# allegro/allRank

Measured on NVIDIA H100. Metric: slates/sec, higher is better.
Workload: dtype tf32

## Files before the change

### allrank_b200/csrc/gemm_tf32.cu

```cuda
#include <cstdio>
#include <cstring>
#include <cuda.h>
#include <cuda_runtime.h>

#include "common.h"
#include "defaults.h"
#include "gemm_tf32.h"
#include "sm90_ptx.cuh"

namespace arb {

constexpr int BLOCK_M = 128;
constexpr int BLOCK_K = 32;
constexpr int BLOCK_K_BF16 = 64;
constexpr int A_STAGE_BYTES = BLOCK_M * BLOCK_K * 4;
constexpr int GEMM_EPI_GROUPS = 1;
constexpr int GEMM_EPI_THREADS = 128 * GEMM_EPI_GROUPS;
constexpr int GEMM_THREADS = 64 + GEMM_EPI_THREADS;
constexpr int XPOSE_BYTES = 32 * 33 * 4;

struct GemmParams {
  int M, N, K;
  int nb2;
  int a_b2, a_b3, b_b2, b_b3, c_b2, c_b3;
// ... 9 lines not shown
  float* colsum_out;
  const int* rows_dev;
  uint32_t* bits;
};

template <bool MN, bool IN16>
__device__ __forceinline__ uint32_t op_word(const uint8_t* s, int rc, int k, int rnd) {
  if constexpr (IN16) {
    if constexpr (MN) {
      const uint8_t* slab = s + (rc >> 6) * 8192;
      const uint32_t lo = *reinterpret_cast<const uint16_t*>(slab + ptx::sw128(k, 2 * (rc & 63)));
      const uint32_t hi = *reinterpret_cast<const uint16_t*>(slab + ptx::sw128(k + 1, 2 * (rc & 63)));
      return lo | (hi << 16);
    } else {
      return *reinterpret_cast<const uint32_t*>(s + ptx::sw128(rc, 2 * k));
    }
  } else {
    const float x = MN ? ptx::ld_f32(s + (rc >> 5) * 4096, k, rc & 31) : ptx::ld_f32(s, rc, k);
    return rnd ? ptx::cvt_tf32(x) : __float_as_uint(x);
  }
}

template <int NT, bool A_MN, bool B_MN, bool IN16>
__device__ __forceinline__ void warp_mma_kblock(float (&acc)[2][NT][4], const uint8_t* a_s, const uint8_t* b_s, int row0,
                                                int slab0, int slab_step, int rnd) {
  const int lane = threadIdx.x & 31, g = lane >> 2, t = lane & 3;
#pragma unroll
  for (int ks = 0; ks < 4; ++ks) {
    const int k0 = IN16 ? 16 * ks + 2 * t : 8 * ks + t;
    const int kh = IN16 ? 8 : 4;
    uint32_t a[2][4];
#pragma unroll
    for (int mt = 0; mt < 2; ++mt) {
      const int r = row0 + 16 * mt + g;
      a[mt][0] = op_word<A_MN, IN16>(a_s, r, k0, rnd);
      a[mt][1] = op_word<A_MN, IN16>(a_s, r + 8, k0, rnd);
      a[mt][2] = op_word<A_MN, IN16>(a_s, r, k0 + kh, rnd);
      a[mt][3] = op_word<A_MN, IN16>(a_s, r + 8, k0 + kh, rnd);
    }
#pragma unroll
    for (int nt = 0; nt < NT; ++nt) {
      const int n = 32 * (slab0 + slab_step * (nt >> 2)) + 8 * (nt & 3) + g;
      const uint32_t b[2] = {op_word<B_MN, IN16>(b_s, n, k0, rnd), op_word<B_MN, IN16>(b_s, n, k0 + kh, rnd)};
#pragma unroll
      for (int mt = 0; mt < 2; ++mt) {
        if constexpr (IN16) ptx::mma_bf16(acc[mt][nt], a[mt], b);
        else ptx::mma_tf32(acc[mt][nt], a[mt], b);
      }
    }
  }
}

template <int A_MN, int B_MN, bool IN16>
constexpr bool use_wgmma() { return A_MN == 0 && B_MN == 0 && !IN16; }
template <int BLOCK_N>
constexpr int wg_cols() { return BLOCK_N == 128 ? 64 : 32; }

template <int NT, int WN>
__device__ __forceinline__ void wg_mma_kblock(float (&acc)[2][NT][4], const uint8_t* a_s, uint8_t* b_s, int col0,
                                              int rnd, int rnd_b, int bar) {
  const int lane = threadIdx.x & 31, w = (threadIdx.x >> 5) & 3, j = lane >> 3;
  if (rnd_b) {
    float4* b4 = reinterpret_cast<float4*>(b_s + col0 * 128);
#pragma unroll
    for (int i = threadIdx.x & 127; i < NT * 8 * 8; i += 128) {
      float4 v = b4[i];
      v.x = __uint_as_float(ptx::cvt_tf32(v.x)); v.y = __uint_as_float(ptx::cvt_tf32(v.y));
      v.z = __uint_as_float(ptx::cvt_tf32(v.z)); v.w = __uint_as_float(ptx::cvt_tf32(v.w));
      b4[i] = v;
    }
    ptx::fence_proxy_async_smem();
    ptx::named_bar_sync(bar, 128);
  }
  uint32_t a[4][2][4];
#pragma unroll
  for (int ks = 0; ks < 4; ++ks)
#pragma unroll
    for (int mt = 0; mt < 2; ++mt) {
      ptx::ldmatrix_x4(a[ks][mt], a_s + ptx::sw128(64 * mt + 16 * w + 8 * (j & 1) + (lane & 7), 32 * ks + 16 * (j >> 1)));
      if (rnd) {
#pragma unroll
        for (int e = 0; e < 4; ++e) a[ks][mt][e] = ptx::cvt_tf32(__uint_as_float(a[ks][mt][e]));
      }
    }
  const uint64_t desc = ptx::wgmma_desc_sw128(b_s + col0 * 128);
  ptx::wgmma_fence_acc(acc[0]);
  ptx::wgmma_fence_acc(acc[1]);
  ptx::wgmma_fence();
#pragma unroll
  for (int ks = 0; ks < 4; ++ks)
#pragma unroll
    for (int mt = 0; mt < 2; ++mt) {
      const uint64_t d = desc + 2 * ks;
      if constexpr (WN == 64) {
        ptx::wgmma_m64n64k8_tf32<0>(acc[mt], a[ks][mt], d);
        if constexpr (NT == 16) ptx::wgmma_m64n64k8_tf32<8>(acc[mt], a[ks][mt], d + 64 * 128 / 16);
      } else {
        ptx::wgmma_m64n32k8_tf32<0>(acc[mt], a[ks][mt], d);
        if constexpr (NT == 8) ptx::wgmma_m64n32k8_tf32<4>(acc[mt], a[ks][mt], d + 32 * 128 / 16);
      }
    }
  ptx::wgmma_commit();
  ptx::wgmma_wait0();
  ptx::wgmma_fence_acc(acc[0]);
  ptx::wgmma_fence_acc(acc[1]);
}

template <int NT>
__device__ __forceinline__ void acc_chunk_row(const float (&acc)[2][NT][4], int c, float* xp, uint32_t (&v)[32]) {
  const int lane = threadIdx.x & 31, g = lane >> 2, t = lane & 3;
  __syncwarp();
#pragma unroll
  for (int cc = 0; cc < NT / 4; ++cc) {
    if (cc != c) continue;
#pragma unroll
    for (int mt = 0; mt < 2; ++mt)
#pragma unroll
      for (int j = 0; j < 4; ++j) {
        float* r0 = xp + (16 * mt + g) * 33 + 8 * j + 2 * t;
        r0[0] = acc[mt][4 * cc + j][0];
        r0[1] = acc[mt][4 * cc + j][1];
        r0[8 * 33] = acc[mt][4 * cc + j][2];
        r0[8 * 33 + 1] = acc[mt][4 * cc + j][3];
      }
  }
  __syncwarp();
#pragma unroll
  for (int j = 0; j < 32; ++j) v[j] = __float_as_uint(xp[lane * 33 + j]);
}

template <int F>
__device__ __forceinline__ uint32_t epi_chunk_f32(const uint32_t (&v)[32], uint8_t* slab_row, int row, const float* bias_c,
                                                  float alpha, uint32_t word = 0u) {
  uint32_t out_bits = 0u;
#pragma unroll
  for (int piece = 0; piece < 8; ++piece) {
    float4* dst = reinterpret_cast<float4*>(slab_row + ((piece ^ (row & 7)) << 4));
    float4 o = make_float4(__uint_as_float(v[piece * 4 + 0]) * alpha, __uint_as_float(v[piece * 4 + 1]) * alpha,
                           __uint_as_float(v[piece * 4 + 2]) * alpha, __uint_as_float(v[piece * 4 + 3]) * alpha);
    if constexpr ((F & EPI_BIAS) != 0) {
      const float4 bv = *reinterpret_cast<const float4*>(bias_c + 4 * piece);
      o.x += bv.x; o.y += bv.y; o.z += bv.z; o.w += bv.w;
    }
    if constexpr ((F & EPI_RELU) != 0) {
      o.x = fmaxf(o.x, 0.0f); o.y = fmaxf(o.y, 0.0f); o.z = fmaxf(o.z, 0.0f); o.w = fmaxf(o.w, 0.0f);
    }
    if constexpr ((F & (EPI_ADD_AUX | EPI_MASK_AUX)) != 0) {
      const float4 a = *dst;
      if constexpr ((F & EPI_ADD_AUX) != 0) { o.x += a.x; o.y += a.y; o.z += a.z; o.w += a.w; }
      if constexpr ((F & EPI_MASK_AUX) != 0) {
        o.x = a.x > 0.f ? o.x : 0.f; o.y = a.y > 0.f ? o.y : 0.f; o.z = a.z > 0.f ? o.z : 0.f; o.w = a.w > 0.f ? o.w : 0.f;
      }
    }
    if constexpr ((F & EPI_MASK_BITS) != 0) {
      o.x = (word >> (4 * piece + 0)) & 1u ? o.x : 0.f; o.y = (word >> (4 * piece + 1)) & 1u ? o.y : 0.f;
      o.z = (word >> (4 * piece + 2)) & 1u ? o.z : 0.f; o.w = (word >> (4 * piece + 3)) & 1u ? o.w : 0.f;
    }
    if constexpr ((F & EPI_RELU_BITS) != 0) {
      out_bits |= (o.x > 0.f ? 1u : 0u) << (4 * piece + 0) | (o.y > 0.f ? 1u : 0u) << (4 * piece + 1) |
                  (o.z > 0.f ? 1u : 0u) << (4 * piece + 2) | (o.w > 0.f ? 1u : 0u) << (4 * piece + 3);
    }
    *dst = o;
  }
  return out_bits;
}
__device__ __forceinline__ bool epi_chunk_dispatch(int flags, const uint32_t (&v)[32], uint8_t* slab_row, int row,
                                                   const float* bias_c, float alpha, uint32_t* bits_at = nullptr,
                                                   uint32_t word_in = 0u) {
  switch (flags & (EPI_BIAS | EPI_RELU | EPI_ADD_AUX | EPI_MASK_AUX | EPI_DROPOUT | EPI_ATOMIC | EPI_RELU_BITS | EPI_MASK_BITS)) {
    case 0: epi_chunk_f32<0>(v, slab_row, row, bias_c, alpha); return true;
    case EPI_BIAS: epi_chunk_f32<EPI_BIAS>(v, slab_row, row, bias_c, alpha); return true;
    case EPI_BIAS | EPI_RELU: epi_chunk_f32<EPI_BIAS | EPI_RELU>(v, slab_row, row, bias_c, alpha); return true;
    case EPI_BIAS | EPI_ADD_AUX: epi_chunk_f32<EPI_BIAS | EPI_ADD_AUX>(v, slab_row, row, bias_c, alpha); return true;
    case EPI_MASK_AUX: epi_chunk_f32<EPI_MASK_AUX>(v, slab_row, row, bias_c, alpha); return true;
    case EPI_BIAS | EPI_RELU | EPI_RELU_BITS: {
      const uint32_t w = epi_chunk_f32<EPI_BIAS | EPI_RELU | EPI_RELU_BITS>(v, slab_row, row, bias_c, alpha);
      if (bits_at) *bits_at = w;
      return true;
    }
    case EPI_MASK_BITS:
      epi_chunk_f32<EPI_MASK_BITS>(v, slab_row, row, bias_c, alpha, word_in);
      return true;
    default: return false;
  }
}

template <int BLOCK_N, int NST = 2>
struct SmemLayout {
  static constexpr int B_STAGE_BYTES = BLOCK_N * BLOCK_K * 4;
  static constexpr int STAGE_BYTES = A_STAGE_BYTES + B_STAGE_BYTES;
  static constexpr int STAGING_BYTES = BLOCK_M * BLOCK_N * 4;
  static constexpr int stages() { return NST; }
  static constexpr int pipe_bytes() { return stages() * STAGE_BYTES; }
  static constexpr int body_bytes() { return pipe_bytes() > STAGING_BYTES ? pipe_bytes() : STAGING_BYTES; }
  static constexpr int XPOSE_OFF = 256 + BLOCK_N * 4;
  static constexpr int total() { return body_bytes() + XPOSE_OFF + (GEMM_EPI_THREADS / 32) * XPOSE_BYTES + 1024; }
};

template <int BLOCK_N, int A_MN, int B_MN, bool DROP, int NST, bool IN16 = false, bool OUT16 = false>
__global__ void __launch_bounds__(GEMM_THREADS) gemm_tf32_kernel(const __grid_constant__ CUtensorMap tmA,
                                                                 const __grid_constant__ CUtensorMap tmB,
                                                                 const __grid_constant__ CUtensorMap tmC,
                                                                 const __grid_constant__ CUtensorMap tmAux,
                                                                 const GemmParams p) {
  using L = SmemLayout<BLOCK_N, NST>;
  constexpr int STAGES = L::stages();
  constexpr int N_SLABS = BLOCK_N / 32;
  constexpr int NT = BLOCK_N / 8;
  constexpr int N_CONSUMERS = GEMM_EPI_THREADS / 32;
  constexpr bool WG = use_wgmma<A_MN, B_MN, IN16>();
  constexpr int OUT_COLS = OUT16 ? 64 : 32;
  constexpr int OUT_SLABS = (BLOCK_N + OUT_COLS - 1) / OUT_COLS;
  static_assert(!OUT16 || BLOCK_N >= 64, "bf16 outputs need at least one full 128-byte slab row");

  extern __shared__ uint8_t smem_dyn[];
  uint8_t* smem = reinterpret_cast<uint8_t*>((reinterpret_cast<uintptr_t>(smem_dyn) + 1023) & ~uintptr_t(1023));
  const bool has_aux = (p.flags & (EPI_ADD_AUX | EPI_MASK_AUX)) != 0;
  uint8_t* staging = smem;
  uint8_t* tail = smem + L::body_bytes();
  uint64_t* full_bar = reinterpret_cast<uint64_t*>(tail);
  uint64_t* empty_bar = full_bar + STAGES;
  uint64_t* ring_done_bar = empty_bar + STAGES;
  uint64_t* aux_bar = ring_done_bar + 1;
  float* bias_s = reinterpret_cast<float*>(tail + 256);

  const int warp = threadIdx.x >> 5, lane = threadIdx.x & 31;
  const int n0 = blockIdx.x * BLOCK_N, m0 = blockIdx.y * BLOCK_M;
  const bool split = (p.flags & EPI_ATOMIC) != 0;
  const int b2 = split ? 0 : int(blockIdx.z) % p.nb2, b3 = split ? 0 : int(blockIdx.z) / p.nb2;
  constexpr int KELEMS = IN16 ? BLOCK_K_BF16 : BLOCK_K;
  constexpr int MN_SLAB = IN16 ? 64 : 32;
  constexpr int MN_SLAB_BYTES = MN_SLAB * KELEMS * (IN16 ? 2 : 4);
  const bool dev_rows = p.rows_dev != nullptr;
  if (dev_rows && !split && m0 >= __ldg(p.rows_dev)) return;
  const int k_live = (dev_rows && split) ? min(p.K, __ldg(p.rows_dev)) : p.K;
  const int total_kb = (k_live + KELEMS - 1) / KELEMS;
  const int kb_per = (dev_rows && split) ? (total_kb + int(gridDim.z) - 1) / int(gridDim.z) : p.kb_per_split;
  const int kb_begin = split ? int(blockIdx.z) * kb_per : 0;
  const int kb_end = split ? min(total_kb, kb_begin + kb_per) : total_kb;
  const int nkb = max(0, kb_end - kb_begin);

  if (warp == 0 && lane == 0) {
    ptx::prefetch_tmap(&tmA);
    ptx::prefetch_tmap(&tmB);
    if (!split) ptx::prefetch_tmap(&tmC);
    if (has_aux) ptx::prefetch_tmap(&tmAux);
    for (int s = 0; s < STAGES; ++s) { ptx::mbar_init(&full_bar[s], 1); ptx::mbar_init(&empty_bar[s], N_CONSUMERS); }
    ptx::mbar_init(ring_done_bar, N_CONSUMERS);
    ptx::mbar_init(aux_bar, 1);
    ptx::fence_barrier_init();
  }
  arb_pdl_wait();
  __syncthreads();

  if (warp == N_CONSUMERS) {
    if (lane == 0) {
      for (int i = 0; i < nkb; ++i) {
        const int s = i % STAGES, round = i / STAGES;
        if (round > 0) ptx::mbar_wait(&empty_bar[s], (round - 1) & 1);
        uint8_t* a_s = smem + s * L::STAGE_BYTES;
        uint8_t* b_s = a_s + A_STAGE_BYTES;
        const int k0 = (kb_begin + i) * KELEMS;
        ptx::mbar_expect_tx(&full_bar[s], L::STAGE_BYTES);
        if (A_MN) {
          for (int c = 0; c < BLOCK_M / MN_SLAB; ++c)
            ptx::tma_load_4d(a_s + c * MN_SLAB_BYTES, &tmA, &full_bar[s], m0 + MN_SLAB * c, k0, b2 * p.a_b2, b3 * p.a_b3);
        } else {
          ptx::tma_load_4d(a_s, &tmA, &full_bar[s], k0, m0, b2 * p.a_b2, b3 * p.a_b3);
        }
        if (B_MN) {
          for (int c = 0; c < BLOCK_N / MN_SLAB; ++c)
            ptx::tma_load_4d(b_s + c * MN_SLAB_BYTES, &tmB, &full_bar[s], n0 + MN_SLAB * c, k0, b2 * p.b_b2, b3 * p.b_b3);
        } else {
          ptx::tma_load_4d(b_s, &tmB, &full_bar[s], k0, n0, b2 * p.b_b2, b3 * p.b_b3);
        }
      }
      if (has_aux) {
        if (nkb > 0) ptx::mbar_wait(ring_done_bar, 0);
        ptx::mbar_expect_tx(aux_bar, OUT16 ? L::STAGING_BYTES / 2 : L::STAGING_BYTES);
        for (int c = 0; c < OUT_SLABS; ++c)
          ptx::tma_load_4d(staging + c * (BLOCK_M * 128), &tmAux, aux_bar, n0 + OUT_COLS * c, m0, b2 * p.c_b2, b3 * p.c_b3);
      }
    }
  } else if (warp < N_CONSUMERS) {
    const int q = warp & 3;
    const int row = WG ? 64 * (lane >> 4) + 16 * q + (lane & 15) : 32 * q + lane;
    const int et = threadIdx.x;
    const int grp = warp >> 2;
    float* xp = reinterpret_cast<float*>(tail + L::XPOSE_OFF) + warp * (XPOSE_BYTES / 4);
    if (p.flags & EPI_BIAS) {
      for (int j = et; j < BLOCK_N; j += GEMM_EPI_THREADS) bias_s[j] = (n0 + j < p.N) ? p.bias[n0 + j] : 0.0f;
    }
    auto mask_word = [&](int c) -> uint32_t {
      return ((p.flags & EPI_MASK_BITS) && c < N_SLABS && m0 + row < p.M && n0 + 32 * c < p.N)
                 ? p.bits[(long long)(m0 + row) * (p.N >> 5) + ((n0 >> 5) + c)] : 0u;
    };
    uint32_t word_next = mask_word(grp);
    float acc[2][NT][4];
#pragma unroll
    for (int mt = 0; mt < 2; ++mt)
#pragma unroll
      for (int nt = 0; nt < NT; ++nt) acc[mt][nt][0] = acc[mt][nt][1] = acc[mt][nt][2] = acc[mt][nt][3] = 0.f;
    for (int i = 0; i < nkb; ++i) {
      const int s = i % STAGES, round = i / STAGES;
      ptx::mbar_wait(&full_bar[s], round & 1);
      uint8_t* a_s = smem + s * L::STAGE_BYTES;
      if constexpr (WG) wg_mma_kblock<NT, wg_cols<BLOCK_N>()>(acc, a_s, a_s + A_STAGE_BYTES, 0, p.rnd, p.rnd_b, 1);
      else warp_mma_kblock<NT, A_MN, B_MN, IN16>(acc, a_s, a_s + A_STAGE_BYTES, 32 * q, 0, 1, p.rnd);
      __syncwarp();
      if (lane == 0) ptx::mbar_arrive(&empty_bar[s]);
    }
    if (lane == 0) ptx::mbar_arrive(ring_done_bar);
    ptx::named_bar_sync(1, GEMM_EPI_THREADS);
    if (has_aux) ptx::mbar_wait(aux_bar, 0);
#pragma unroll 1
    for (int c = grp; c < N_SLABS; c += GEMM_EPI_GROUPS) {
      const uint32_t word_in = word_next;
      word_next = mask_word(c + GEMM_EPI_GROUPS);
      uint32_t v[32];
      acc_chunk_row<NT>(acc, c, xp, v);
      if constexpr (OUT16) {
        uint8_t* slab_row = staging + (c >> 1) * (BLOCK_M * 128) + row * 128;
#pragma unroll
        for (int piece = 0; piece < 4; ++piece) {
          uint4* dst = reinterpret_cast<uint4*>(slab_row + ((((c & 1) * 4 + piece) ^ (row & 7)) << 4));
          float o[8];
#pragma unroll
          for (int e = 0; e < 8; ++e) {
            const int j = piece * 8 + e;
            float x = __uint_as_float(v[j]) * p.alpha;
            if (p.flags & EPI_BIAS) x += bias_s[32 * c + j];
            if (p.flags & EPI_RELU) x = fmaxf(x, 0.0f);
            if constexpr (DROP) {
              const unsigned long long idx = (unsigned long long)(m0 + row) * (unsigned long long)p.N + (n0 + 32 * c + j);
              x = drop_keep(idx, p.drop.seed, p.drop.thresh) ? x * p.drop.scale : 0.0f;
            }
            o[e] = x;
          }
          if (has_aux) {
            const uint4 a = *dst;
            const uint32_t w[4] = {a.x, a.y, a.z, a.w};
#pragma unroll
            for (int e = 0; e < 8; ++e) {
              const uint32_t h = (w[e >> 1] >> ((e & 1) * 16)) & 0xffffu;
              const float av = __uint_as_float(h << 16);
              if (p.flags & EPI_ADD_AUX) o[e] += av;
              if (p.flags & EPI_MASK_AUX) o[e] = av > 0.f ? o[e] : 0.f;
            }
          }
          uint4 pk;
          pk.x = ptx::pack_bf16(o[0], o[1]); pk.y = ptx::pack_bf16(o[2], o[3]);
          pk.z = ptx::pack_bf16(o[4], o[5]); pk.w = ptx::pack_bf16(o[6], o[7]);
          *dst = pk;
        }
        continue;
      }
      uint8_t* slab_row = staging + c * (BLOCK_M * 128) + row * 128;
      if constexpr (!DROP) {
        uint32_t* bits_at = (p.bits && m0 + row < p.M && n0 + 32 * c < p.N)
                                ? p.bits + (long long)(m0 + row) * (p.N >> 5) + ((n0 >> 5) + c) : nullptr;
        if (epi_chunk_dispatch(p.flags, v, slab_row, row, bias_s + 32 * c, p.alpha, bits_at, word_in)) continue;
      }
#pragma unroll
// ... 51 lines not shown
          const uint8_t* slab = staging + (et >> 6) * (BLOCK_M * 128);
          const int cc = et & 63;
#pragma unroll 8
          for (int r = 0; r < BLOCK_M; ++r) {
            const uint16_t hv = *reinterpret_cast<const uint16_t*>(slab + r * 128 + ((((cc >> 3) ^ (r & 7)) << 4) | ((cc & 7) << 1)));
            t += __uint_as_float(uint32_t(hv) << 16);
          }
        } else {
          const uint8_t* slab = staging + (et >> 5) * (BLOCK_M * 128);
          const int cc = et & 31;
#pragma unroll 8
          for (int r = 0; r < BLOCK_M; ++r)
            t += *reinterpret_cast<const float*>(slab + r * 128 + ((((cc >> 2) ^ (r & 7)) << 4) | ((cc & 3) << 2)));
        }
        p.colsum_out[((long long)blockIdx.z * gridDim.y + blockIdx.y) * p.N + n0 + et] = t;
      }
      if (et == 0) ptx::tma_store_wait_read();
    }
  }
  __syncthreads();
}

template <int BLOCK_N>
struct PersistLayout {
  static constexpr int B_STAGE_BYTES = BLOCK_N * BLOCK_K * 4;
  static constexpr int STAGE_BYTES = A_STAGE_BYTES + B_STAGE_BYTES;
  static constexpr int STAGES = BLOCK_N <= 64 ? 6 : 3;
  static constexpr int STAGING_BYTES = BLOCK_M * BLOCK_N * 4;
  static constexpr int RING_BYTES = STAGES * STAGE_BYTES;
  static constexpr int XPOSE_OFF = RING_BYTES + STAGING_BYTES + 512 + BLOCK_N * 4;
  static constexpr int total();
};

constexpr int EPI_GROUPS = 2;
constexpr int EPI_THREADS = 128 * EPI_GROUPS;
constexpr int PERSIST_THREADS = 64 + EPI_THREADS;
template <int BLOCK_N>
constexpr int PersistLayout<BLOCK_N>::total() { return XPOSE_OFF + (EPI_THREADS / 32) * XPOSE_BYTES + 1024; }

template <int BLOCK_N, int A_MN, int B_MN>
__global__ void __launch_bounds__(PERSIST_THREADS, 1) gemm_tf32_persistent(const __grid_constant__ CUtensorMap tmA,
                                                                        const __grid_constant__ CUtensorMap tmB,
                                                                        const __grid_constant__ CUtensorMap tmC,
                                                                        const __grid_constant__ CUtensorMap tmAux,
                                                                        const GemmParams p, int n_tiles_n,
                                                                        int n_tiles_m, int n_z) {
  using L = PersistLayout<BLOCK_N>;
  constexpr int STAGES = L::STAGES;
  constexpr int N_SLABS = BLOCK_N / 32;
  constexpr int NGA = N_SLABS < EPI_GROUPS ? N_SLABS : EPI_GROUPS;
  constexpr int SLABS_PER_GROUP = N_SLABS / NGA;
  constexpr int NT = 4 * SLABS_PER_GROUP;
  constexpr bool WG = use_wgmma<A_MN, B_MN, false>();
  static_assert(!WG || 32 * SLABS_PER_GROUP == wg_cols<BLOCK_N>(), "a group's columns are one wgmma instruction wide");
  constexpr int PRODUCER_WARP = EPI_THREADS / 32;

  extern __shared__ uint8_t smem_dyn[];
  uint8_t* smem = reinterpret_cast<uint8_t*>((reinterpret_cast<uintptr_t>(smem_dyn) + 1023) & ~uintptr_t(1023));
  uint8_t* staging = smem + L::RING_BYTES;
  uint64_t* full_bar = reinterpret_cast<uint64_t*>(staging + L::STAGING_BYTES);
  uint64_t* empty_bar = full_bar + STAGES;
  uint64_t* aux_full = empty_bar + STAGES;
  uint64_t* stage_free = aux_full + 1;
  float* bias_s = reinterpret_cast<float*>(staging + L::STAGING_BYTES + 512);

  const int warp = threadIdx.x >> 5, lane = threadIdx.x & 31;
  const bool split = (p.flags & EPI_ATOMIC) != 0;
  const bool has_aux = (p.flags & (EPI_ADD_AUX | EPI_MASK_AUX)) != 0;
  const bool dev_rows = p.rows_dev != nullptr;
  if (dev_rows && !split) n_tiles_m = min(n_tiles_m, (__ldg(p.rows_dev) + BLOCK_M - 1) / BLOCK_M);
  const int total_kb = (((dev_rows && split) ? min(p.K, __ldg(p.rows_dev)) : p.K) + BLOCK_K - 1) / BLOCK_K;
  const int kb_per = (dev_rows && split) ? (total_kb + n_z - 1) / n_z : p.kb_per_split;
  const int n_tiles = n_tiles_n * n_tiles_m * n_z;

  if (warp == 0 && lane == 0) {
    ptx::prefetch_tmap(&tmA);
    ptx::prefetch_tmap(&tmB);
    if (!split) ptx::prefetch_tmap(&tmC);
    if (has_aux) ptx::prefetch_tmap(&tmAux);
    for (int s = 0; s < STAGES; ++s) { ptx::mbar_init(&full_bar[s], 1); ptx::mbar_init(&empty_bar[s], 4 * NGA); }
    ptx::mbar_init(aux_full, 1);
    ptx::mbar_init(stage_free, NGA);
    ptx::fence_barrier_init();
  }
  arb_pdl_wait();
  __syncthreads();

  auto decode = [&](int t, int& n0, int& m0, int& z) {
    const int nt = t % n_tiles_n;
    const int rest = t / n_tiles_n;
    n0 = nt * BLOCK_N;
    m0 = (rest % n_tiles_m) * BLOCK_M;
    z = rest / n_tiles_m;
  };
  auto k_range = [&](int z, int& kb0, int& nkb) {
    if (split) {
      kb0 = z * kb_per;
      nkb = min(total_kb, kb0 + kb_per) - kb0;
      if (nkb < 0) nkb = 0;
    } else {
      kb0 = 0;
      nkb = total_kb;
    }
  };

  if (warp == PRODUCER_WARP) {
// ... 238 lines not shown
static int launch_persistent_t(const GemmDesc& d, const CUtensorMap& tA, const CUtensorMap& tB, const CUtensorMap& tC,
                               const CUtensorMap& tX, const GemmParams& p, dim3 tiles, cudaStream_t st) {
  const long long n_tiles = (long long)tiles.x * tiles.y * tiles.z;
  const int grid = int(std::min<long long>(n_tiles, sm_count()));
  const double nb = double(d.nb2) * double(d.nb3);
  const double has_x = (d.flags & (EPI_ADD_AUX | EPI_MASK_AUX)) ? 1.0 : 0.0;
  char pname[56];
  gemm_prof_name(pname, d, "persist");
  const double dM = live_m(d), dK = live_k(d);
  ProfScope ps(ARB_PROF_GEMM, 2.0 * dM * double(d.N) * dK * nb, st,
               4.0 * nb * (dM * dK + double(d.N) * dK + (1.0 + has_x) * dM * d.N), pname);
  return launch(gemm_tf32_persistent<BLOCK_N, A_MN, B_MN>, dim3(grid), dim3(PERSIST_THREADS),
                PersistLayout<BLOCK_N>::total(), st, true, tA, tB, tC, tX, p, int(tiles.x), int(tiles.y),
                int(tiles.z));
}

template <int BLOCK_N, int A_MN, int B_MN>
static int launch_bf16_t(const GemmDesc& d, const CUtensorMap& tA, const CUtensorMap& tB, const CUtensorMap& tC,
                         const CUtensorMap& tX, const GemmParams& p, dim3 grid, cudaStream_t st) {
  constexpr bool WGRAD = (A_MN == 1 && B_MN == 1);
  const bool drop = (p.flags & EPI_DROPOUT) != 0;
  if (drop && (A_MN || B_MN)) { arb_set_error("gemm_bf16: dropout epilogue needs K-major operands"); return ARB_E_UNSUPPORTED; }
  void (*kern)(CUtensorMap, CUtensorMap, CUtensorMap, CUtensorMap, GemmParams) = nullptr;
  int smem = 0;
  if constexpr (WGRAD) {
    kern = gemm_tf32_kernel<BLOCK_N, 1, 1, false, 4, true, false>; smem = SmemLayout<BLOCK_N, 4>::total();
  } else if constexpr (BLOCK_N >= 64) {
    constexpr bool CAN_DROP = (A_MN == 0 && B_MN == 0);
    if (d.C.bf16) {
      if (drop) kern = gemm_tf32_kernel<BLOCK_N, A_MN, B_MN, CAN_DROP, 3, true, true>;
      else      kern = gemm_tf32_kernel<BLOCK_N, A_MN, B_MN, false, 3, true, true>;
    } else {
      if (drop) kern = gemm_tf32_kernel<BLOCK_N, A_MN, B_MN, CAN_DROP, 3, true, false>;
      else      kern = gemm_tf32_kernel<BLOCK_N, A_MN, B_MN, false, 3, true, false>;
    }
    smem = SmemLayout<BLOCK_N, 3>::total();
  }
  if (!kern) { arb_set_error("gemm_bf16: block_n must be 64 or 128"); return ARB_E_UNSUPPORTED; }
  const double nb = double(d.nb2) * double(d.nb3);
  const double has_x = (d.flags & (EPI_ADD_AUX | EPI_MASK_AUX)) ? 1.0 : 0.0;
  const double osz = d.C.bf16 ? 2.0 : 4.0;
  char pname[56];
  gemm_prof_name(pname, d, "tile");
  const double dM = live_m(d), dK = live_k(d);
  ProfScope ps(ARB_PROF_GEMM, 2.0 * dM * double(d.N) * dK * nb, st,
               nb * (2.0 * (dM * dK + double(d.N) * dK) + osz * (1.0 + has_x) * dM * d.N), pname);
  return launch(kern, grid, dim3(GEMM_THREADS), smem, st, true, tA, tB, tC, tX, p);
}

template <int BLOCK_N, int A_MN, int B_MN>
static int launch_t(const GemmDesc& d, const CUtensorMap& tA, const CUtensorMap& tB, const CUtensorMap& tC,
                    const CUtensorMap& tX, const GemmParams& p, dim3 grid, cudaStream_t st) {
  if (d.A.bf16) return launch_bf16_t<BLOCK_N, A_MN, B_MN>(d, tA, tB, tC, tX, p, grid, st);
  const bool has_aux_tile = (p.flags & (EPI_ADD_AUX | EPI_MASK_AUX)) != 0;
  const bool pick = !(A_MN == 1 && B_MN == 1) && !(p.flags & EPI_ATOMIC) && d.nb2 == 1 && d.nb3 == 1 &&
                    (d.K >= 256 || !has_aux_tile || g_persistent == 3);
  if (g_persistent == 1 || (g_persistent >= 2 && pick))
    return launch_persistent_t<BLOCK_N, A_MN, B_MN>(d, tA, tB, tC, tX, p, grid, st);
  constexpr bool CAN_DROP = (A_MN == 0 && B_MN == 0);
  constexpr bool WGRAD = (A_MN == 1 && B_MN == 1);
  const bool drop = (p.flags & EPI_DROPOUT) != 0;
  if (drop && !CAN_DROP) { arb_set_error("gemm_tf32: dropout epilogue needs K-major operands"); return ARB_E_UNSUPPORTED; }
  const bool deep = !WGRAD && d.K >= 256;
  void (*kern)(CUtensorMap, CUtensorMap, CUtensorMap, CUtensorMap, GemmParams);
  int smem;
  if (WGRAD) {
    kern = gemm_tf32_kernel<BLOCK_N, A_MN, B_MN, false, 4>; smem = SmemLayout<BLOCK_N, 4>::total();
  } else if (drop) {
    if (deep) { kern = gemm_tf32_kernel<BLOCK_N, A_MN, B_MN, CAN_DROP, 3>; smem = SmemLayout<BLOCK_N, 3>::total(); }
    else      { kern = gemm_tf32_kernel<BLOCK_N, A_MN, B_MN, CAN_DROP, 2>; smem = SmemLayout<BLOCK_N, 2>::total(); }
  } else {
    if (deep) { kern = gemm_tf32_kernel<BLOCK_N, A_MN, B_MN, false, 3>; smem = SmemLayout<BLOCK_N, 3>::total(); }
    else      { kern = gemm_tf32_kernel<BLOCK_N, A_MN, B_MN, false, 2>; smem = SmemLayout<BLOCK_N, 2>::total(); }
  }
  const double nb = double(d.nb2) * double(d.nb3);
  const double has_x = (d.flags & (EPI_ADD_AUX | EPI_MASK_AUX)) ? 1.0 : 0.0;
  char pname[56];
  gemm_prof_name(pname, d, "tile");
  const double dM = live_m(d), dK = live_k(d);
  ProfScope ps(ARB_PROF_GEMM, 2.0 * dM * double(d.N) * dK * nb, st,
               4.0 * nb * (dM * dK + double(d.N) * dK + (1.0 + has_x) * dM * d.N), pname);
  return launch(kern, grid, dim3(GEMM_THREADS), smem, st, true, tA, tB, tC, tX, p);
}

int launch_gemm_tf32(const GemmDesc& d, cudaStream_t st) {
  if (d.M <= 0 || d.N <= 0 || d.K < 0) { arb_set_error("gemm_tf32: bad shape"); return ARB_E_INVALID_ARG; }
  if (d.block_n != 32 && d.block_n != 64 && d.block_n != 128) { arb_set_error("gemm_tf32: block_n must be 32/64/128"); return ARB_E_INVALID_ARG; }
  const bool split = (d.flags & EPI_ATOMIC) != 0;
  if (split && (d.nb2 != 1 || d.nb3 != 1 || !d.atomic_out)) { arb_set_error("gemm_tf32: split-K needs an unbatched problem and atomic_out"); return ARB_E_INVALID_ARG; }
  if (!split && d.split_k != 1) { arb_set_error("gemm_tf32: split_k > 1 needs EPI_ATOMIC"); return ARB_E_INVALID_ARG; }
  const bool in16 = d.A.bf16 != 0, out16 = d.C.bf16 != 0;
  if ((d.B.bf16 != 0) != in16) { arb_set_error("gemm: A and B must have the same element type"); return ARB_E_INVALID_ARG; }
  if (out16 && (!in16 || split || d.block_n < 64)) { arb_set_error("gemm: a bf16 output needs bf16 operands, no split-K and block_n >= 64"); return ARB_E_INVALID_ARG; }
  if ((d.flags & (EPI_ADD_AUX | EPI_MASK_AUX)) && (d.Aux.bf16 != 0) != out16) { arb_set_error("gemm: the aux tile must have the output's element type"); return ARB_E_INVALID_ARG; }
  if (in16 && d.block_n < 64) { arb_set_error("gemm: bf16 operands need block_n >= 64 (a 128-byte row holds 64 elements)"); return ARB_E_INVALID_ARG; }
  if (in16 && (d.nb2 != 1 || d.nb3 != 1)) { arb_set_error("gemm: bf16 operands serve the unbatched linears only"); return ARB_E_UNSUPPORTED; }
  const uint32_t kel = in16 ? 64u : 32u;
  const uint32_t ocol = out16 ? 64u : 32u;
  alignas(64) CUtensorMap tA, tB, tC, tX;
  int rc;
  if ((rc = make_tmap_4d(&tA, d.A, d.a_mn ? TmapBox{{kel, kel, 1, 1}} : TmapBox{{kel, 128, 1, 1}}, 0))) return rc;
  if ((rc = make_tmap_4d(&tB, d.B, d.b_mn ? TmapBox{{kel, kel, 1, 1}} : TmapBox{{kel, uint32_t(d.block_n), 1, 1}}, 0))) return rc;
  if (!split) {
    if ((rc = make_tmap_4d(&tC, d.C, TmapBox{{ocol, 128, 1, 1}}, 0))) return rc;
  } else {
    tC = tA;
  }
  if (d.flags & (EPI_ADD_AUX | EPI_MASK_AUX)) {
    if ((rc = make_tmap_4d(&tX, d.Aux, TmapBox{{ocol, 128, 1, 1}}, 0))) return rc;
  } else {
    tX = tA;
  }
  const int total_kb = (d.K + int(kel) - 1) / int(kel);
  const int splits = split ? std::max(1, std::min(d.split_k, total_kb)) : 1;
  GemmParams p;
  p.M = d.M; p.N = d.N; p.K = d.K; p.nb2 = d.nb2;
  p.a_b2 = d.a_b2; p.a_b3 = d.a_b3; p.b_b2 = d.b_b2; p.b_b3 = d.b_b3; p.c_b2 = d.c_b2; p.c_b3 = d.c_b3;
  p.flags = d.flags; p.alpha = d.alpha; p.bias = d.bias; p.atomic_out = d.atomic_out; p.atomic_ld = d.atomic_ld;
  p.drop = d.drop;
  p.colsum_out = d.colsum_out;
// ... 86 lines not shown
```

### allrank_b200/csrc/sm90_ptx.cuh

```cuda
#pragma once
#include <cstdint>
#include <cuda.h>
#include <cuda_runtime.h>

namespace arb {
namespace ptx {

__device__ __forceinline__ uint32_t smem_u32(const void* p) {
  return static_cast<uint32_t>(__cvta_generic_to_shared(p));
}

__device__ __forceinline__ void mbar_init(uint64_t* bar, uint32_t count) {
  asm volatile("mbarrier.init.shared::cta.b64 [%0], %1;" ::"r"(smem_u32(bar)), "r"(count) : "memory");
}
__device__ __forceinline__ void fence_barrier_init() {
  asm volatile("fence.mbarrier_init.release.cluster;" ::: "memory");
}
__device__ __forceinline__ void mbar_expect_tx(uint64_t* bar, uint32_t bytes) {
  asm volatile("mbarrier.arrive.expect_tx.shared::cta.b64 _, [%0], %1;" ::"r"(smem_u32(bar)), "r"(bytes) : "memory");
}
__device__ __forceinline__ void mbar_arrive(uint64_t* bar) {
  asm volatile("mbarrier.arrive.shared::cta.b64 _, [%0];" ::"r"(smem_u32(bar)) : "memory");
}
__device__ __forceinline__ bool mbar_try_wait(uint64_t* bar, uint32_t parity) {
  uint32_t ok;
  asm volatile(
      "{\n\t.reg .pred p;\n\t"
      "mbarrier.try_wait.parity.shared::cta.b64 p, [%1], %2;\n\t"
      "selp.u32 %0, 1, 0, p;\n\t}"
      : "=r"(ok)
      : "r"(smem_u32(bar)), "r"(parity)
      : "memory");
  return ok != 0;
}
__device__ __forceinline__ void mbar_wait(uint64_t* bar, uint32_t parity) {
  if (mbar_try_wait(bar, parity)) return;
  const long long t0 = clock64();
  while (!mbar_try_wait(bar, parity)) {
    if (clock64() - t0 > 4000000000LL) __trap();
  }
}

__device__ __forceinline__ void fence_proxy_async_smem() {
  asm volatile("fence.proxy.async.shared::cta;" ::: "memory");
}
__device__ __forceinline__ void named_bar_sync(uint32_t id, uint32_t nthreads) {
  asm volatile("bar.sync %0, %1;" ::"r"(id), "r"(nthreads) : "memory");
}

__device__ __forceinline__ void prefetch_tmap(const CUtensorMap* m) {
  asm volatile("prefetch.tensormap [%0];" ::"l"(reinterpret_cast<uint64_t>(m)) : "memory");
}
__device__ __forceinline__ void tma_load_4d(void* dst, const CUtensorMap* m, uint64_t* bar, int c0, int c1, int c2,
                                            int c3) {
  asm volatile(
      "cp.async.bulk.tensor.4d.shared::cluster.global.mbarrier::complete_tx::bytes [%0], [%1, {%3, %4, %5, %6}], [%2];"
      ::"r"(smem_u32(dst)), "l"(reinterpret_cast<uint64_t>(m)), "r"(smem_u32(bar)), "r"(c0), "r"(c1), "r"(c2), "r"(c3)
      : "memory");
}
__device__ __forceinline__ void tma_store_4d(const CUtensorMap* m, const void* src, int c0, int c1, int c2, int c3) {
  asm volatile("cp.async.bulk.tensor.4d.global.shared::cta.bulk_group [%0, {%2, %3, %4, %5}], [%1];"
               ::"l"(reinterpret_cast<uint64_t>(m)), "r"(smem_u32(src)), "r"(c0), "r"(c1), "r"(c2), "r"(c3)
               : "memory");
}
__device__ __forceinline__ void tma_store_commit() { asm volatile("cp.async.bulk.commit_group;" ::: "memory"); }
__device__ __forceinline__ void tma_store_wait_all() { asm volatile("cp.async.bulk.wait_group 0;" ::: "memory"); }
__device__ __forceinline__ void tma_store_wait_read() { asm volatile("cp.async.bulk.wait_group.read 0;" ::: "memory"); }

__device__ __forceinline__ uint32_t pack_bf16(float lo, float hi) {
  uint32_t r;
  asm("cvt.rn.bf16x2.f32 %0, %1, %2;" : "=r"(r) : "f"(hi), "f"(lo));
  return r;
}

__device__ __forceinline__ uint32_t sw128(int r, int b) {
  return uint32_t(r) * 128u + ((uint32_t((b >> 4) ^ (r & 7))) << 4) + uint32_t(b & 15);
}
__device__ __forceinline__ float ld_f32(const uint8_t* tile, int r, int c) {
  return *reinterpret_cast<const float*>(tile + sw128(r, 4 * c));
}

__device__ __forceinline__ uint32_t cvt_tf32(float x) {
  uint32_t r;
  asm("cvt.rn.tf32.f32 %0, %1;" : "=r"(r) : "f"(x));
  return r;
}
__device__ __forceinline__ void mma_tf32(float (&d)[4], const uint32_t (&a)[4], const uint32_t (&b)[2]) {
  asm volatile(
      "mma.sync.aligned.m16n8k8.row.col.f32.tf32.tf32.f32 {%0, %1, %2, %3}, {%4, %5, %6, %7}, {%8, %9}, "
      "{%0, %1, %2, %3};"
      : "+f"(d[0]), "+f"(d[1]), "+f"(d[2]), "+f"(d[3])
      : "r"(a[0]), "r"(a[1]), "r"(a[2]), "r"(a[3]), "r"(b[0]), "r"(b[1]));
}
__device__ __forceinline__ void mma_bf16(float (&d)[4], const uint32_t (&a)[4], const uint32_t (&b)[2]) {
  asm volatile(
      "mma.sync.aligned.m16n8k16.row.col.f32.bf16.bf16.f32 {%0, %1, %2, %3}, {%4, %5, %6, %7}, {%8, %9}, "
      "{%0, %1, %2, %3};"
      : "+f"(d[0]), "+f"(d[1]), "+f"(d[2]), "+f"(d[3])
      : "r"(a[0]), "r"(a[1]), "r"(a[2]), "r"(a[3]), "r"(b[0]), "r"(b[1]));
}
__device__ __forceinline__ void ldmatrix_x4(uint32_t (&r)[4], const void* row_addr) {
  asm volatile("ldmatrix.sync.aligned.m8n8.x4.shared.b16 {%0, %1, %2, %3}, [%4];"
               : "=r"(r[0]), "=r"(r[1]), "=r"(r[2]), "=r"(r[3])
               : "r"(smem_u32(row_addr)));
}

__device__ __forceinline__ uint64_t wgmma_desc_sw128(const void* tile) {
  const uint64_t addr = smem_u32(tile);
  return ((addr & 0x3FFFFull) >> 4) | (uint64_t(1) << 16) | (uint64_t(1024 >> 4) << 32) | (uint64_t(1) << 62);
}
__device__ __forceinline__ void wgmma_fence() { asm volatile("wgmma.fence.sync.aligned;" ::: "memory"); }
__device__ __forceinline__ void wgmma_commit() { asm volatile("wgmma.commit_group.sync.aligned;" ::: "memory"); }
__device__ __forceinline__ void wgmma_wait0() { asm volatile("wgmma.wait_group.sync.aligned 0;" ::: "memory"); }
template <int NT>
__device__ __forceinline__ void wgmma_fence_acc(float (&d)[NT][4]) {
#pragma unroll
  for (int j = 0; j < NT; ++j) asm volatile("" : "+f"(d[j][0]), "+f"(d[j][1]), "+f"(d[j][2]), "+f"(d[j][3])::"memory");
}

#define ARB_D4(j) "+f"(d[J0 + j][0]), "+f"(d[J0 + j][1]), "+f"(d[J0 + j][2]), "+f"(d[J0 + j][3])
template <int J0, int NT>
__device__ __forceinline__ void wgmma_m64n32k8_tf32(float (&d)[NT][4], const uint32_t (&a)[4], uint64_t desc_b) {
  asm volatile(
      "{\n\t.reg .pred p;\n\tsetp.ne.b32 p, %21, 0;\n\t"
      "wgmma.mma_async.sync.aligned.m64n32k8.f32.tf32.tf32 "
      "{%0, %1, %2, %3, %4, %5, %6, %7, %8, %9, %10, %11, %12, %13, %14, %15}, "
      "{%16, %17, %18, %19}, %20, p, 1, 1;\n\t}"
      : ARB_D4(0), ARB_D4(1), ARB_D4(2), ARB_D4(3)
      : "r"(a[0]), "r"(a[1]), "r"(a[2]), "r"(a[3]), "l"(desc_b), "r"(1));
}
template <int J0, int NT>
__device__ __forceinline__ void wgmma_m64n64k8_tf32(float (&d)[NT][4], const uint32_t (&a)[4], uint64_t desc_b) {
  asm volatile(
      "{\n\t.reg .pred p;\n\tsetp.ne.b32 p, %37, 0;\n\t"
      "wgmma.mma_async.sync.aligned.m64n64k8.f32.tf32.tf32 "
      "{%0, %1, %2, %3, %4, %5, %6, %7, %8, %9, %10, %11, %12, %13, %14, %15, "
      "%16, %17, %18, %19, %20, %21, %22, %23, %24, %25, %26, %27, %28, %29, %30, %31}, "
      "{%32, %33, %34, %35}, %36, p, 1, 1;\n\t}"
      : ARB_D4(0), ARB_D4(1), ARB_D4(2), ARB_D4(3), ARB_D4(4), ARB_D4(5), ARB_D4(6), ARB_D4(7)
      : "r"(a[0]), "r"(a[1]), "r"(a[2]), "r"(a[3]), "l"(desc_b), "r"(1));
}
#undef ARB_D4

__device__ __forceinline__ void acc_to_a_tf32(const float (&c)[4], uint32_t (&a)[4], int lane) {
  const int t = lane & 3, base = lane & ~3;
  const int s1 = base + (t >> 1), s2 = base + 2 + (t >> 1);
  const float x0 = __shfl_sync(0xffffffffu, c[0], s1), x1 = __shfl_sync(0xffffffffu, c[1], s1);
  const float y0 = __shfl_sync(0xffffffffu, c[2], s1), y1 = __shfl_sync(0xffffffffu, c[3], s1);
  const float u0 = __shfl_sync(0xffffffffu, c[0], s2), u1 = __shfl_sync(0xffffffffu, c[1], s2);
  const float w0 = __shfl_sync(0xffffffffu, c[2], s2), w1 = __shfl_sync(0xffffffffu, c[3], s2);
  const bool odd = (t & 1) != 0;
  a[0] = __float_as_uint(odd ? x1 : x0);
  a[1] = __float_as_uint(odd ? y1 : y0);
  a[2] = __float_as_uint(odd ? u1 : u0);
  a[3] = __float_as_uint(odd ? w1 : w0);
}

}
}
```

Baseline: 174,200.

## Use wgmma for weight-gradient GEMMs via in-smem K-major transpose

For the case where both operands are MN-major (weight gradients), the consumer warpgroup now transposes each pipeline stage in shared memory into a K-major swizzled buffer, applying optional tf32 rounding, and issues shared-memory-descriptor wgmma instead of mma.sync. A double-buffered K-major area lets the transpose of the next stage overlap the async wgmma of the previous one. The cost is extra shared memory traffic and footprint per stage, plus a named barrier per k-block. The persistent-kernel path is now skipped at compile time for this case.

```diff
diff --git a/allrank_b200/csrc/gemm_tf32.cu b/allrank_b200/csrc/gemm_tf32.cu
--- a/allrank_b200/csrc/gemm_tf32.cu
+++ b/allrank_b200/csrc/gemm_tf32.cu
@@ -85,7 +85,9 @@
 }
 
 template <int A_MN, int B_MN, bool IN16>
-constexpr bool use_wgmma() { return A_MN == 0 && B_MN == 0 && !IN16; }
+constexpr bool use_wgmma() { return A_MN == B_MN && !IN16; }
+template <int A_MN, int B_MN, bool IN16>
+constexpr bool wgmma_transposed() { return A_MN == 1 && B_MN == 1 && !IN16; }
 template <int BLOCK_N>
 constexpr int wg_cols() { return BLOCK_N == 128 ? 64 : 32; }
 
@@ -137,6 +139,62 @@
   ptx::wgmma_wait0();
   ptx::wgmma_fence_acc(acc[0]);
   ptx::wgmma_fence_acc(acc[1]);
+}
+
+template <int NSLAB>
+__device__ __forceinline__ void wg_kmajor_stage(const uint8_t* ring, uint8_t* kt, int rnd) {
+  constexpr int TASKS = 8 * NSLAB, PER = (TASKS + 15) / 16;
+  const int l = threadIdx.x & 7, grp = (threadIdx.x & 127) >> 3;
+  const uint32_t src0 = ptx::smem_u32(ring), dst0 = ptx::smem_u32(kt);
+  float v[PER][4][4];
+#pragma unroll
+  for (int u = 0; u < PER; ++u) {
+    const int task = grp + 16 * u;
+    if (TASKS % 16 != 0 && task >= TASKS) continue;
+    const uint32_t src = src0 + (task >> 3) * 4096;
+    const int c = l ^ (task & 7);
+#pragma unroll
+    for (int j = 0; j < 4; ++j) {
+      const int k = 4 * l + j;
+      const float4 x = ptx::lds128(src + k * 128 + ((c ^ (k & 7)) << 4));
+      v[u][j][0] = x.x; v[u][j][1] = x.y; v[u][j][2] = x.z; v[u][j][3] = x.w;
+    }
+  }
+#pragma unroll
+  for (int u = 0; u < PER; ++u) {
+    const int task = grp + 16 * u;
+    if (TASKS % 16 != 0 && task >= TASKS) continue;
+    const uint32_t dst = dst0 + (task >> 3) * 4096;
+    const int c = l ^ (task & 7);
+#pragma unroll
+    for (int j = 0; j < 4; ++j) {
+      const int m = 4 * c + j;
+      float o[4];
+#pragma unroll
+      for (int e = 0; e < 4; ++e) o[e] = rnd ? __uint_as_float(ptx::cvt_tf32(v[u][e][j])) : v[u][e][j];
+      ptx::sts128(dst + m * 128 + ((l ^ (m & 7)) << 4), make_float4(o[0], o[1], o[2], o[3]));
+    }
+  }
+}
+
+template <int NT, int WN>
+__device__ __forceinline__ void wg_mma_kmajor(float (&acc)[2][NT][4], const uint8_t* kt) {
+  const uint64_t da = ptx::wgmma_desc_sw128(kt), db = ptx::wgmma_desc_sw128(kt + A_STAGE_BYTES);
+  ptx::wgmma_fence();
+#pragma unroll
+  for (int ks = 0; ks < 4; ++ks)
+#pragma unroll
+    for (int mt = 0; mt < 2; ++mt) {
+      const uint64_t a = da + mt * (64 * 128 / 16) + 2 * ks, b = db + 2 * ks;
+      if constexpr (WN == 64) {
+        ptx::wgmma_m64n64k8_tf32_ss<0>(acc[mt], a, b);
+        if constexpr (NT == 16) ptx::wgmma_m64n64k8_tf32_ss<8>(acc[mt], a, b + 64 * 128 / 16);
+      } else {
+        ptx::wgmma_m64n32k8_tf32_ss<0>(acc[mt], a, b);
+        if constexpr (NT == 8) ptx::wgmma_m64n32k8_tf32_ss<4>(acc[mt], a, b + 32 * 128 / 16);
+      }
+    }
+  ptx::wgmma_commit();
 }
 
 template <int NT>
@@ -218,14 +276,17 @@
   }
 }
 
-template <int BLOCK_N, int NST = 2>
+template <int BLOCK_N, int NST = 2, bool KM = false>
 struct SmemLayout {
   static constexpr int B_STAGE_BYTES = BLOCK_N * BLOCK_K * 4;
   static constexpr int STAGE_BYTES = A_STAGE_BYTES + B_STAGE_BYTES;
   static constexpr int STAGING_BYTES = BLOCK_M * BLOCK_N * 4;
   static constexpr int stages() { return NST; }
   static constexpr int pipe_bytes() { return stages() * STAGE_BYTES; }
-  static constexpr int body_bytes() { return pipe_bytes() > STAGING_BYTES ? pipe_bytes() : STAGING_BYTES; }
+  static constexpr int kmajor_bytes() { return KM ? 2 * STAGE_BYTES : 0; }
+  static constexpr int body_bytes() {
+    return pipe_bytes() + kmajor_bytes() > STAGING_BYTES ? pipe_bytes() + kmajor_bytes() : STAGING_BYTES;
+  }
   static constexpr int XPOSE_OFF = 256 + BLOCK_N * 4;
   static constexpr int total() { return body_bytes() + XPOSE_OFF + (GEMM_EPI_THREADS / 32) * XPOSE_BYTES + 1024; }
 };
@@ -236,12 +297,14 @@
                                                                  const __grid_constant__ CUtensorMap tmC,
                                                                  const __grid_constant__ CUtensorMap tmAux,
                                                                  const GemmParams p) {
-  using L = SmemLayout<BLOCK_N, NST>;
+  constexpr bool WG = use_wgmma<A_MN, B_MN, IN16>();
+  constexpr bool WG_T = wgmma_transposed<A_MN, B_MN, IN16>();
+  using L = SmemLayout<BLOCK_N, NST, WG_T>;
   constexpr int STAGES = L::stages();
   constexpr int N_SLABS = BLOCK_N / 32;
   constexpr int NT = BLOCK_N / 8;
   constexpr int N_CONSUMERS = GEMM_EPI_THREADS / 32;
-  constexpr bool WG = use_wgmma<A_MN, B_MN, IN16>();
+  static_assert(!WG_T || N_CONSUMERS == 4, "the K-major rewrite is one warpgroup's");
   constexpr int OUT_COLS = OUT16 ? 64 : 32;
   constexpr int OUT_SLABS = (BLOCK_N + OUT_COLS - 1) / OUT_COLS;
   static_assert(!OUT16 || BLOCK_N >= 64, "bf16 outputs need at least one full 128-byte slab row");
@@ -334,14 +397,35 @@
     for (int mt = 0; mt < 2; ++mt)
 #pragma unroll
       for (int nt = 0; nt < NT; ++nt) acc[mt][nt][0] = acc[mt][nt][1] = acc[mt][nt][2] = acc[mt][nt][3] = 0.f;
-    for (int i = 0; i < nkb; ++i) {
-      const int s = i % STAGES, round = i / STAGES;
-      ptx::mbar_wait(&full_bar[s], round & 1);
-      uint8_t* a_s = smem + s * L::STAGE_BYTES;
-      if constexpr (WG) wg_mma_kblock<NT, wg_cols<BLOCK_N>()>(acc, a_s, a_s + A_STAGE_BYTES, 0, p.rnd, p.rnd_b, 1);
-      else warp_mma_kblock<NT, A_MN, B_MN, IN16>(acc, a_s, a_s + A_STAGE_BYTES, 32 * q, 0, 1, p.rnd);
-      __syncwarp();
-      if (lane == 0) ptx::mbar_arrive(&empty_bar[s]);
+    if constexpr (WG_T) {
+      uint8_t* kmajor = smem + L::pipe_bytes();
+      for (int i = 0; i < nkb; ++i) {
+        const int s = i % STAGES, round = i / STAGES;
+        ptx::mbar_wait(&full_bar[s], round & 1);
+        uint8_t* kt = kmajor + (i & 1) * L::STAGE_BYTES;
+        wg_kmajor_stage<4 + N_SLABS>(smem + s * L::STAGE_BYTES, kt, p.rnd);
+        ptx::fence_proxy_async_smem();
+        __syncwarp();
+        if (lane == 0) ptx::mbar_arrive(&empty_bar[s]);
+        ptx::wgmma_wait0();
+        ptx::wgmma_fence_acc(acc[0]);
+        ptx::wgmma_fence_acc(acc[1]);
+        ptx::named_bar_sync(1, GEMM_EPI_THREADS);
+        wg_mma_kmajor<NT, wg_cols<BLOCK_N>()>(acc, kt);
+      }
+      ptx::wgmma_wait0();
+      ptx::wgmma_fence_acc(acc[0]);
+      ptx::wgmma_fence_acc(acc[1]);
+    } else {
+      for (int i = 0; i < nkb; ++i) {
+        const int s = i % STAGES, round = i / STAGES;
+        ptx::mbar_wait(&full_bar[s], round & 1);
+        uint8_t* a_s = smem + s * L::STAGE_BYTES;
+        if constexpr (WG) wg_mma_kblock<NT, wg_cols<BLOCK_N>()>(acc, a_s, a_s + A_STAGE_BYTES, 0, p.rnd, p.rnd_b, 1);
+        else warp_mma_kblock<NT, A_MN, B_MN, IN16>(acc, a_s, a_s + A_STAGE_BYTES, 32 * q, 0, 1, p.rnd);
+        __syncwarp();
+        if (lane == 0) ptx::mbar_arrive(&empty_bar[s]);
+      }
     }
     if (lane == 0) ptx::mbar_arrive(ring_done_bar);
     ptx::named_bar_sync(1, GEMM_EPI_THREADS);
@@ -499,6 +583,7 @@
   constexpr int SLABS_PER_GROUP = N_SLABS / NGA;
   constexpr int NT = 4 * SLABS_PER_GROUP;
   constexpr bool WG = use_wgmma<A_MN, B_MN, false>();
+  static_assert(!wgmma_transposed<A_MN, B_MN, false>(), "both operands MN-major: one-tile kernel only");
   static_assert(!WG || 32 * SLABS_PER_GROUP == wg_cols<BLOCK_N>(), "a group's columns are one wgmma instruction wide");
   constexpr int PRODUCER_WARP = EPI_THREADS / 32;
 
@@ -843,20 +928,22 @@
 static int launch_t(const GemmDesc& d, const CUtensorMap& tA, const CUtensorMap& tB, const CUtensorMap& tC,
                     const CUtensorMap& tX, const GemmParams& p, dim3 grid, cudaStream_t st) {
   if (d.A.bf16) return launch_bf16_t<BLOCK_N, A_MN, B_MN>(d, tA, tB, tC, tX, p, grid, st);
-  const bool has_aux_tile = (p.flags & (EPI_ADD_AUX | EPI_MASK_AUX)) != 0;
-  const bool pick = !(A_MN == 1 && B_MN == 1) && !(p.flags & EPI_ATOMIC) && d.nb2 == 1 && d.nb3 == 1 &&
-                    (d.K >= 256 || !has_aux_tile || g_persistent == 3);
-  if (g_persistent == 1 || (g_persistent >= 2 && pick))
-    return launch_persistent_t<BLOCK_N, A_MN, B_MN>(d, tA, tB, tC, tX, p, grid, st);
+  constexpr bool WGRAD = (A_MN == 1 && B_MN == 1);
+  if constexpr (!WGRAD) {
+    const bool has_aux_tile = (p.flags & (EPI_ADD_AUX | EPI_MASK_AUX)) != 0;
+    const bool pick = !(p.flags & EPI_ATOMIC) && d.nb2 == 1 && d.nb3 == 1 &&
+                      (d.K >= 256 || !has_aux_tile || g_persistent == 3);
+    if (g_persistent == 1 || (g_persistent >= 2 && pick))
+      return launch_persistent_t<BLOCK_N, A_MN, B_MN>(d, tA, tB, tC, tX, p, grid, st);
+  }
   constexpr bool CAN_DROP = (A_MN == 0 && B_MN == 0);
-  constexpr bool WGRAD = (A_MN == 1 && B_MN == 1);
   const bool drop = (p.flags & EPI_DROPOUT) != 0;
   if (drop && !CAN_DROP) { arb_set_error("gemm_tf32: dropout epilogue needs K-major operands"); return ARB_E_UNSUPPORTED; }
   const bool deep = !WGRAD && d.K >= 256;
   void (*kern)(CUtensorMap, CUtensorMap, CUtensorMap, CUtensorMap, GemmParams);
   int smem;
-  if (WGRAD) {
-    kern = gemm_tf32_kernel<BLOCK_N, A_MN, B_MN, false, 4>; smem = SmemLayout<BLOCK_N, 4>::total();
+  if constexpr (WGRAD) {
+    kern = gemm_tf32_kernel<BLOCK_N, A_MN, B_MN, false, 4>; smem = SmemLayout<BLOCK_N, 4, true>::total();
   } else if (drop) {
     if (deep) { kern = gemm_tf32_kernel<BLOCK_N, A_MN, B_MN, CAN_DROP, 3>; smem = SmemLayout<BLOCK_N, 3>::total(); }
     else      { kern = gemm_tf32_kernel<BLOCK_N, A_MN, B_MN, CAN_DROP, 2>; smem = SmemLayout<BLOCK_N, 2>::total(); }
diff --git a/allrank_b200/csrc/sm90_ptx.cuh b/allrank_b200/csrc/sm90_ptx.cuh
--- a/allrank_b200/csrc/sm90_ptx.cuh
+++ b/allrank_b200/csrc/sm90_ptx.cuh
@@ -76,6 +76,14 @@
 __device__ __forceinline__ uint32_t sw128(int r, int b) {
   return uint32_t(r) * 128u + ((uint32_t((b >> 4) ^ (r & 7))) << 4) + uint32_t(b & 15);
 }
+__device__ __forceinline__ float4 lds128(uint32_t addr) {
+  float4 v;
+  asm volatile("ld.shared.v4.f32 {%0, %1, %2, %3}, [%4];" : "=f"(v.x), "=f"(v.y), "=f"(v.z), "=f"(v.w) : "r"(addr));
+  return v;
+}
+__device__ __forceinline__ void sts128(uint32_t addr, float4 v) {
+  asm volatile("st.shared.v4.f32 [%0], {%1, %2, %3, %4};" ::"r"(addr), "f"(v.x), "f"(v.y), "f"(v.z), "f"(v.w) : "memory");
+}
 __device__ __forceinline__ float ld_f32(const uint8_t* tile, int r, int c) {
   return *reinterpret_cast<const float*>(tile + sw128(r, 4 * c));
 }
@@ -140,6 +148,27 @@
       : ARB_D4(0), ARB_D4(1), ARB_D4(2), ARB_D4(3), ARB_D4(4), ARB_D4(5), ARB_D4(6), ARB_D4(7)
       : "r"(a[0]), "r"(a[1]), "r"(a[2]), "r"(a[3]), "l"(desc_b), "r"(1));
 }
+template <int J0, int NT>
+__device__ __forceinline__ void wgmma_m64n32k8_tf32_ss(float (&d)[NT][4], uint64_t desc_a, uint64_t desc_b) {
+  asm volatile(
+      "{\n\t.reg .pred p;\n\tsetp.ne.b32 p, %18, 0;\n\t"
+      "wgmma.mma_async.sync.aligned.m64n32k8.f32.tf32.tf32 "
+      "{%0, %1, %2, %3, %4, %5, %6, %7, %8, %9, %10, %11, %12, %13, %14, %15}, "
+      "%16, %17, p, 1, 1;\n\t}"
+      : ARB_D4(0), ARB_D4(1), ARB_D4(2), ARB_D4(3)
+      : "l"(desc_a), "l"(desc_b), "r"(1));
+}
+template <int J0, int NT>
+__device__ __forceinline__ void wgmma_m64n64k8_tf32_ss(float (&d)[NT][4], uint64_t desc_a, uint64_t desc_b) {
+  asm volatile(
+      "{\n\t.reg .pred p;\n\tsetp.ne.b32 p, %34, 0;\n\t"
+      "wgmma.mma_async.sync.aligned.m64n64k8.f32.tf32.tf32 "
+      "{%0, %1, %2, %3, %4, %5, %6, %7, %8, %9, %10, %11, %12, %13, %14, %15, "
+      "%16, %17, %18, %19, %20, %21, %22, %23, %24, %25, %26, %27, %28, %29, %30, %31}, "
+      "%32, %33, p, 1, 1;\n\t}"
+      : ARB_D4(0), ARB_D4(1), ARB_D4(2), ARB_D4(3), ARB_D4(4), ARB_D4(5), ARB_D4(6), ARB_D4(7)
+      : "l"(desc_a), "l"(desc_b), "r"(1));
+}
 #undef ARB_D4
 
 __device__ __forceinline__ void acc_to_a_tf32(const float (&c)[4], uint32_t (&a)[4], int lane) {
```

After: 188,900, median of 6. 8.4% higher.
